# huggingface/parler-tts

Measured on NVIDIA H100. Metric: audio codec tokens/sec (all codebooks), higher is better.
Workload: dtype bf16

## Files before the change

include/ptts_b200.h:

```cpp
#ifndef PTTS_B200_H
#define PTTS_B200_H

#include <stdint.h>

#ifdef __cplusplus
extern "C" {
#endif

#define PTTS_OK 0
#define PTTS_EINVAL 1
#define PTTS_ECUDA 2
#define PTTS_ESTATE 3

#define PTTS_BF16 0
#define PTTS_F32 1
#define PTTS_I64 2
#define PTTS_I32 3

#define PTTS_HEAD_DIM 64

typedef struct ptts_decoder_config {
  int32_t hidden_size;
  int32_t num_layers;
  int32_t num_heads;
// ... 89 lines not shown
               float* out_token_nll, float* out_logits, float* out_codebook_sums, void* stream);

int ptts_decode_forward(ptts_session* s, void* stream);

int ptts_sample(ptts_session* s, const int64_t* forced_tokens, void* stream);

int ptts_decode_steps(ptts_session* s, int32_t n_steps, void* stream);

int ptts_generate_set_sampling_ext(ptts_session* s, const ptts_sampling_ext* ext);

int ptts_generate_set_outputs(ptts_session* s, float* logits, float* scores, int32_t first_step, int32_t n_steps,
                              int64_t step_stride);

int ptts_generate_set_probes(ptts_session* s, void* self_attn, void* cross_attn, void* hidden, int32_t first_step, int32_t n_steps,
                             int64_t self_ld, int64_t self_step, int64_t cross_step, int64_t hidden_step);

int ptts_session_logits(ptts_session* s, float** out);
int ptts_session_scores(ptts_session* s, float** out);
int ptts_session_raw_ids(ptts_session* s, int64_t** out, int32_t* ld);
int ptts_session_state(ptts_session* s, int32_t** out);
int ptts_session_launches(ptts_session* s, int64_t* out);
int ptts_session_fused(ptts_session* s, int32_t* out);
int ptts_session_set_profile(ptts_session* s, void* buf);

int ptts_delay_build(const int64_t* input_ids, int32_t BK, int32_t seq_len, int32_t num_codebooks,
                     int64_t bos, int64_t pad, int32_t max_length, int64_t* pattern_mask, void* stream);
int ptts_delay_apply(const int64_t* input_ids, int32_t BK, int32_t seq_len, int64_t ld_ids,
                     const int64_t* pattern_mask, int64_t ld_mask, int64_t* out, void* stream);
int ptts_logits_processor(const int64_t* input_ids, int32_t BK, int32_t seq_len, int64_t ld_ids,
                          float* scores, int32_t V, int64_t eos, int32_t num_codebooks,
                          int64_t* first_unfinished, void* stream);
int ptts_op_sample_phase(ptts_session* s, int32_t n_ctas, void* stream);
int ptts_op_linear2(const ptts_decoder_config* cfg, const void* blob, int32_t tensor_id, int32_t index,
                    const void* x, int32_t M, int32_t use_ln, int32_t epilogue ,
                    const void* residual, void* y, int32_t path, float* row_stats, void* stream);
int ptts_op_linear(const ptts_decoder_config* cfg, const void* blob, int32_t tensor_id, int32_t index,
                   const void* x, int32_t M, int32_t use_ln, int32_t epilogue, const void* residual, void* y, void* stream);
int ptts_op_attention(int32_t dtype, int32_t B, int32_t nh, int32_t nkv, int32_t q_len, int32_t past_len, int32_t cross,
                      int32_t kv_len, int32_t capacity, int32_t rope, const void* rope_cos, const void* rope_sin, const void* qkv,
                      void* kcache, void* vcache, const int32_t* key_mask, int32_t mask_len, int32_t prefill_sweep, void* out,
                      void* stream);

int ptts_op_attention_probs(int32_t dtype, int32_t B, int32_t nh, int32_t nkv, int32_t q_len, int32_t past_len, int32_t cross,
                            int32_t kv_len, int32_t capacity, int32_t rope, const void* rope_cos, const void* rope_sin, const void* q,
                            int64_t ldq, const void* kcache, const int32_t* key_mask, int32_t mask_len, void* out, void* stream);

// ... 34 lines not shown
```

parler_tts_b200/_lib.py:

```python
from __future__ import annotations
import ctypes as C
import os

import torch

_HERE = os.path.dirname(os.path.abspath(__file__))
LIB_PATH = os.environ.get("PTTS_LIB") or os.path.join(_HERE, "csrc", "libptts_b200.so")

BF16, F32, I64, I32 = 0, 1, 2, 3
OK, EINVAL, ECUDA, ESTATE = 0, 1, 2, 3


class DecoderConfigC(C.Structure):
    _fields_ = [(n, C.c_int32) for n in (
        "hidden_size", "num_layers", "num_heads", "num_kv_heads", "num_cross_kv_heads", "ffn_dim", "vocab_size",
        "num_codebooks", "max_positions", "rope", "activation", "dtype", "bos_token_id", "pad_token_id",
        "eos_token_id")] + [("rope_theta", C.c_float), ("layer_norm_eps", C.c_float)]


class GenParamsC(C.Structure):
    _fields_ = [("max_length", C.c_int32), ("min_new_tokens", C.c_int32), ("do_sample", C.c_int32),
                ("top_k", C.c_int32), ("top_p", C.c_float), ("temperature", C.c_float), ("seed", C.c_uint64),
                ("suppress_special", C.c_int32), ("codebook_size", C.c_int32),
                ("row_base", C.c_int32), ("input_len", C.c_int32)]
# ... 26 lines not shown
    "ptts_session_create": (C.c_int, [C.POINTER(DecoderConfigC), _VP, _VP, _I64, _I32, _I32, _I32, _I32, C.POINTER(_VP)]),
    "ptts_workspace_bytes2": (C.c_int, [C.POINTER(DecoderConfigC), _I32, _I32, _I32, _I32, _I32, C.POINTER(_I64)]),
    "ptts_session_create2": (C.c_int, [C.POINTER(DecoderConfigC), _VP, _VP, _I64, _I32, _I32, _I32, _I32, _I32, C.POINTER(_VP)]),
    "ptts_session_destroy": (C.c_int, [_VP]),
    "ptts_generate_begin": (C.c_int, [_VP, C.POINTER(GenParamsC), _VP]),
    "ptts_generate_begin_ids": (C.c_int, [_VP, C.POINTER(GenParamsC), _VP, _I32, _VP]),
    "ptts_generate_set_sampling_ext": (C.c_int, [_VP, C.POINTER(SamplingExtC)]),
    "ptts_generate_set_outputs": (C.c_int, [_VP, _VP, _VP, _I32, _I32, _I64]),
    "ptts_generate_set_probes": (C.c_int, [_VP, _VP, _VP, _VP, _I32, _I32, _I64, _I64, _I64, _I64]),
    "ptts_prefill": (C.c_int, [_VP, _VP, _VP, _VP, _VP, _VP]),
    "ptts_lm_heads_rowmajor_bytes": (C.c_int, [C.POINTER(DecoderConfigC), C.POINTER(_I64)]),
    "ptts_lm_heads_rowmajor_pack": (C.c_int, [C.POINTER(DecoderConfigC), _VP, _VP, _VP]),
    "ptts_score": (C.c_int, [_VP, _VP, _VP, _VP, _VP, _VP, _VP, _I32, _VP, _VP, _VP, _VP, _VP]),
    "ptts_decode_forward": (C.c_int, [_VP, _VP]),
    "ptts_sample": (C.c_int, [_VP, _VP, _VP]),
    "ptts_decode_steps": (C.c_int, [_VP, _I32, _VP]),
    "ptts_session_logits": (C.c_int, [_VP, C.POINTER(_VP)]),
    "ptts_session_scores": (C.c_int, [_VP, C.POINTER(_VP)]),
    "ptts_session_raw_ids": (C.c_int, [_VP, C.POINTER(_VP), C.POINTER(_I32)]),
    "ptts_session_state": (C.c_int, [_VP, C.POINTER(_VP)]),
    "ptts_session_launches": (C.c_int, [_VP, C.POINTER(_I64)]),
    "ptts_session_fused": (C.c_int, [_VP, C.POINTER(_I32)]),
    "ptts_session_set_profile": (C.c_int, [_VP, _VP]),
    "ptts_delay_build": (C.c_int, [_VP, _I32, _I32, _I32, _I64, _I64, _I32, _VP, _VP]),
    "ptts_delay_apply": (C.c_int, [_VP, _I32, _I32, _I64, _VP, _I64, _VP, _VP]),
    "ptts_logits_processor": (C.c_int, [_VP, _I32, _I32, _I64, _VP, _I32, _I64, _I32, _VP, _VP]),
    "ptts_op_sample_phase": (C.c_int, [_VP, _I32, _VP]),
    "ptts_op_linear": (C.c_int, [C.POINTER(DecoderConfigC), _VP, _I32, _I32, _VP, _I32, _I32, _I32, _VP, _VP, _VP]),
    "ptts_op_linear2": (C.c_int, [C.POINTER(DecoderConfigC), _VP, _I32, _I32, _VP, _I32, _I32, _I32, _VP, _VP, _I32, _VP, _VP]),
    "ptts_op_attention": (C.c_int, [_I32, _I32, _I32, _I32, _I32, _I32, _I32, _I32, _I32, _I32, _VP, _VP, _VP, _VP, _VP, _VP,
                                    _I32, _I32, _VP, _VP]),
    "ptts_op_attention_probs": (C.c_int, [_I32, _I32, _I32, _I32, _I32, _I32, _I32, _I32, _I32, _I32, _VP, _VP, _VP, _I64, _VP,
                                          _VP, _I32, _VP, _VP]),
    "ptts_dac_blob_bytes": (C.c_int, [C.POINTER(DacConfigC), C.POINTER(_I64)]),
    "ptts_dac_num_tensors": (C.c_int, [C.POINTER(DacConfigC), C.POINTER(_I32)]),
    "ptts_dac_pack": (C.c_int, [C.POINTER(DacConfigC), _VP, _I32, _VP, _I32, _I64, _VP]),
    "ptts_dac_workspace_bytes": (C.c_int, [C.POINTER(DacConfigC), _I32, _I32, C.POINTER(_I64)]),
    "ptts_dac_decode": (C.c_int, [C.POINTER(DacConfigC), _VP, _VP, _I64, _VP, _I32, _I32, _VP, _VP]),
    "ptts_dac_encoder_blob_bytes": (C.c_int, [C.POINTER(DacConfigC), C.POINTER(_I64)]),
    "ptts_dac_encoder_num_tensors": (C.c_int, [C.POINTER(DacConfigC), C.POINTER(_I32)]),
    "ptts_dac_encoder_pack": (C.c_int, [C.POINTER(DacConfigC), _VP, _I32, _VP, _I32, _I64, _VP]),
    "ptts_dac_encode_workspace_bytes": (C.c_int, [C.POINTER(DacConfigC), _I32, _I32, C.POINTER(_I64)]),
    "ptts_dac_encode": (C.c_int, [C.POINTER(DacConfigC), _VP, _VP, _VP, _I64, _VP, _I32, _I32, _I32, _VP, _VP, _VP]),
}
EXPORTED_SYMBOLS = tuple(_SIGS)

# ... 52 lines not shown
```

parler_tts_b200/csrc/api.cu:

```cuda
#include <cstdarg>
#include <cstdlib>
#include <cstring>
#include <new>

#include "common.cuh"
#include "dac.h"
#include "kernels.h"
#include "layout.h"
#include "step.h"

namespace ptts {
static thread_local std::string g_err;
void set_error(const std::string& m) { g_err = m; }
int fail(int code, const char* fmt, ...) {
  char buf[1024];
  va_list ap;
  va_start(ap, fmt);
  vsnprintf(buf, sizeof(buf), fmt, ap);
  va_end(ap);
  g_err = buf;
  return code;
}
static bool env_flag(const char* name, bool dflt) {
  const char* v = getenv(name);
// ... 11 lines not shown
};

struct ProbeWindow {
  void* self_attn; void* cross_attn; void* hidden;
  int first_step, n_steps;
  int64_t self_ld, self_step, cross_step, hidden_step;
};

struct ptts_session {
  ptts_decoder_config cfg;
  DecoderLayout L;
  WorkspaceLayout W;
  const char* blob;
  char* ws;
  int sm_count;
  bool has_prompt_mask, has_enc_mask, begun, prefilled;
  ptts_gen_params gen;
  int n0;
  cudaStream_t cap_stream;
  cudaGraphExec_t exec;
  bool graph_ready;
  int64_t launches;
  long long* prof;
  DecodePath path;
  StepParams sp;
  ptts_sampling_ext ext;
  SampleOut out;
  ProbeWindow probe;
  int64_t graph_launches;
};

static const ptts_sampling_ext kExtOff = {0, 0.f, 1.f, 0.f, 0.f};
static const ptts_sampling_ext* active_ext(const ptts_session* s) {
  const ptts_sampling_ext& x = s->ext;
  const bool warp = s->gen.do_sample && (x.min_p > 0.f || x.typical_p < 1.f || x.epsilon_cutoff > 0.f || x.eta_cutoff > 0.f);
  return (x.no_repeat_ngram_size > 0 || warp) ? &s->ext : nullptr;
}
static const SampleOut* active_out(const ptts_session* s) {
  return (s->out.logits != nullptr || s->out.scores != nullptr) ? &s->out : nullptr;
}
static const ProbeWindow* active_probe(const ptts_session* s) {
  const ProbeWindow& w = s->probe;
  return (w.self_attn != nullptr || w.cross_attn != nullptr || w.hidden != nullptr) ? &w : nullptr;
}
static DecodePath decode_path(const ptts_session* s) { return active_probe(s) != nullptr ? DECODE_MULTI_KERNEL : s->path; }

// ... 201 lines not shown
  const WorkspaceLayout& W = s->W;
  if (c.dtype != PTTS_BF16 || !env_flag("PTTS_FUSED", true)) return DECODE_MULTI_KERNEL;
  if (W.B > 32 || L.K > 16 || L.H % 64 != 0 || L.F % L.H != 0) return step_declined(s, "batch > 32 rows, > 16 codebooks or an unsupported width");
  StepParams& p = s->sp;
  memset(&p, 0, sizeof(p));
  p.B = W.B; p.H = L.H; p.F = L.F; p.V = L.V; p.K = L.K; p.L = L.L; p.nh = L.nh; p.nkv = L.nkv; p.nckv = L.nckv;
  p.S = W.S; p.P = W.P; p.Tmax = W.Tmax; p.rope = c.rope; p.act = c.activation; p.qkv_rows = L.qkv_rows; p.ckv_rows = L.ckv_rows;
  p.eps = c.layer_norm_eps; p.scale = 0.125f;
  p.blob = s->blob;
  p.lay = L;
  char* ws = s->ws;
  p.x = (bf16*)(ws + W.img_x); p.qkv = (bf16*)(ws + W.qkv); p.attn = (bf16*)(ws + W.img_attn); p.qc = (bf16*)(ws + W.qc); p.hbuf = (bf16*)(ws + W.img_h);
  p.logits = (float*)(ws + W.logits);
  p.cross_kv = ws + W.cross_kv; p.cross_layer_stride = W.cross_layer_stride;
  p.self_kv = ws + W.self_kv; p.self_layer_stride = W.self_layer_stride;
  p.prompt_mask = s->has_prompt_mask ? (const int*)(ws + W.prompt_mask) : nullptr;
  p.enc_mask = s->has_enc_mask ? (const int*)(ws + W.enc_mask) : nullptr;
  p.sa = sample_args(s);
  p.bar = ((Ctrl*)(ws + W.ctrl))->bar;
  p.progress = (int*)(ws + W.progress);
  if (const char* why = plan_decode_step(p, s->sm_count)) return step_declined(s, why);
  p.do_sample_phase = 1;
  p.prof = s->prof;
  p.cl_x = (bf16*)(ws + W.cl_x); p.cl_attn = (bf16*)(ws + W.cl_attn); p.cl_h = (bf16*)(ws + W.cl_h);
  const char* mode = getenv("PTTS_STEP");
  if (L.cl_NC > 0 && !(mode && strcmp(mode, "legacy") == 0) && cluster_step_available(p)) return DECODE_CLUSTER;
  return DECODE_STEP;
}

int ptts_generate_begin_ids(ptts_session* s, const ptts_gen_params* gen, const int64_t* input_ids, int32_t n0, void* stream) {
  PTTS_REQUIRE(s && gen, "null argument");
  PTTS_REQUIRE(n0 >= 1 && n0 <= s->W.max_input, "generate: %d decoder input columns, the session takes 1 .. %d", n0, s->W.max_input);
  PTTS_REQUIRE(input_ids != nullptr || n0 == 1, "generate: input_ids is required for %d input columns", n0);
  PTTS_REQUIRE(gen->max_length >= 2, "generate: max_length must be >= 2, got %d", gen->max_length);
  PTTS_REQUIRE(gen->max_length <= s->W.raw_ld, "generate: max_length %d exceeds the session's capacity %lld", gen->max_length, (long long)s->W.raw_ld);
  PTTS_REQUIRE(!gen->do_sample || gen->temperature > 0.f, "`temperature` has to be a strictly positive float, got %f", gen->temperature);
  PTTS_REQUIRE(gen->top_k >= 0, "`top_k` has to be a non-negative integer");
  PTTS_REQUIRE(s->cfg.eos_token_id >= 0 && s->cfg.eos_token_id < s->cfg.vocab_size, "eos_token_id out of vocabulary");
  PTTS_REQUIRE(n0 < gen->max_length, "generate: %d input columns leave nothing to generate within max_length %d", n0, gen->max_length);
  cudaStream_t st = (cudaStream_t)stream;
  s->gen = *gen;
  s->gen.input_len = n0;
  s->n0 = n0;
  s->ext = kExtOff;
  s->out = SampleOut{};
  if (active_probe(s) && s->exec) { cudaGraphExecDestroy(s->exec); s->exec = nullptr; s->graph_ready = false; }
// ... 375 lines not shown
    ce = cudaGraphInstantiate(&s->exec, graph, 0);
    cudaGraphDestroy(graph);
    if (ce != cudaSuccess) return fail(PTTS_ECUDA, "graph instantiate failed: %s", cudaGetErrorString(ce));
    s->graph_ready = true;
  }
  for (int i = 0; i < n_steps; i++) PTTS_CHECK_CUDA(cudaGraphLaunch(s->exec, st));
  s->launches += s->graph_launches * n_steps;
  return PTTS_OK;
}

int ptts_session_logits(ptts_session* s, float** out) { PTTS_REQUIRE(s && out, "null"); *out = (float*)(s->ws + s->W.logits); return PTTS_OK; }
int ptts_session_scores(ptts_session* s, float** out) { PTTS_REQUIRE(s && out, "null"); *out = (float*)(s->ws + s->W.scores); return PTTS_OK; }
int ptts_session_raw_ids(ptts_session* s, int64_t** out, int32_t* ld) {
  PTTS_REQUIRE(s && out && ld, "null");
  *out = (int64_t*)(s->ws + s->W.raw_ids);
  *ld = (int32_t)s->W.raw_ld;
  return PTTS_OK;
}
int ptts_session_state(ptts_session* s, int32_t** out) { PTTS_REQUIRE(s && out, "null"); *out = (int32_t*)(s->ws + s->W.ctrl); return PTTS_OK; }
int ptts_session_set_profile(ptts_session* s, void* buf) {
  PTTS_REQUIRE(s, "null");
  s->prof = (long long*)buf;
  s->sp.prof = s->prof;
  return PTTS_OK;
}
int ptts_session_fused(ptts_session* s, int32_t* out) { PTTS_REQUIRE(s && out, "null"); *out = s->path; return PTTS_OK; }
int ptts_session_launches(ptts_session* s, int64_t* out) { PTTS_REQUIRE(s && out, "null"); *out = s->launches; return PTTS_OK; }

int ptts_delay_build(const int64_t* input_ids, int32_t BK, int32_t seq_len, int32_t num_codebooks, int64_t bos, int64_t pad,
                     int32_t max_length, int64_t* pattern_mask, void* stream) {
  PTTS_REQUIRE(input_ids && pattern_mask, "null argument");
  PTTS_REQUIRE(num_codebooks > 0 && BK > 0 && BK % num_codebooks == 0 && seq_len > 0 && max_length > 0, "delay_build: bad shape");
  return launch_delay_build(input_ids, BK, seq_len, num_codebooks, bos, pad, max_length, pattern_mask, (cudaStream_t)stream);
}
int ptts_delay_apply(const int64_t* input_ids, int32_t BK, int32_t seq_len, int64_t ld_ids, const int64_t* pattern_mask,
                     int64_t ld_mask, int64_t* out, void* stream) {
  PTTS_REQUIRE(input_ids && pattern_mask && out, "null argument");
  PTTS_REQUIRE(BK > 0 && seq_len > 0 && ld_mask >= seq_len && ld_ids >= seq_len, "delay_apply: mask shorter than ids");
  return launch_delay_apply(input_ids, BK, seq_len, ld_ids, pattern_mask, ld_mask, out, (cudaStream_t)stream);
}
int ptts_logits_processor(const int64_t* input_ids, int32_t BK, int32_t seq_len, int64_t ld_ids, float* scores, int32_t V,
                          int64_t eos, int32_t num_codebooks, int64_t* first_unfinished, void* stream) {
  PTTS_REQUIRE(input_ids && scores && first_unfinished, "null argument");
  return launch_logits_processor(input_ids, BK, seq_len, ld_ids, scores, V, eos, num_codebooks, first_unfinished, (cudaStream_t)stream);
}

// ... 406 lines not shown
```

parler_tts_b200/csrc/sample_core.cuh:

```cuda
#pragma once
#include "common.cuh"
#include "kernels.h"

namespace ptts {

__device__ __forceinline__ uint32_t fkey(float f) {
  uint32_t u = __float_as_uint(f);
  return (u & 0x80000000u) ? ~u : (u | 0x80000000u);
}

__device__ __forceinline__ void philox_round(uint32_t (&c)[4], uint32_t k0, uint32_t k1) {
  const uint32_t hi0 = __umulhi(0xD2511F53u, c[0]), lo0 = 0xD2511F53u * c[0];
  const uint32_t hi1 = __umulhi(0xCD9E8D57u, c[2]), lo1 = 0xCD9E8D57u * c[2];
  c[0] = hi1 ^ c[1] ^ k0; c[1] = lo1; c[2] = hi0 ^ c[3] ^ k1; c[3] = lo0;
}
__device__ __forceinline__ float philox_uniform(uint64_t seed, uint32_t row, uint32_t col) {
  uint32_t c[4] = {row, col, 0x5054u, 0x5453u};
  uint32_t k0 = (uint32_t)seed, k1 = (uint32_t)(seed >> 32);
#pragma unroll
  for (int i = 0; i < 10; i++) { philox_round(c, k0, k1); k0 += 0x9E3779B9u; k1 += 0xBB67AE85u; }
  return (float)(c[0] >> 8) * (1.0f / 16777216.0f);
}


// ... 434 lines not shown
    const int still_unfinished = t_unf && !done;
    p.unfinished[my_row] = still_unfinished;
    int nxt = t;
    if (g.max_length >= 2 * p.K - 1) {
      const bool is_bos = cur_len <= k;
      const bool is_pad = (cur_len - k) >= (g.max_length - p.K + 1);
      if (is_bos || is_pad) nxt = (is_bos ? p.bos : 0) + (is_pad ? p.pad : 0);
      else if (g.input_len > 1 && cur_len - g.input_len < k) nxt = (int)p.prefix_cells[(size_t)my_row * (p.K - 1) + (cur_len - g.input_len)];
    }
    p.cur_ids[my_row] = nxt;
    if (still_unfinished) atomicAdd(&p.ctrl->n_unfinished, 1);
  }
  __syncthreads();
}

template <int ITEMS>
__device__ __forceinline__ void sample_row_cta(const SampleArgs& p, const ptts_gen_params& g, const int64_t* __restrict__ forced,
                                               int row, int cur_len) {
  sample_rows_cta<ITEMS, 1>(p, g, forced, row, 0, row + 1, cur_len);
}

template <int ITEMS>
__device__ __forceinline__ void sample_all_rows_cta(const SampleArgs& p, const ptts_gen_params& g, int cta, int n_ctas, int n_rows, int cur_len) {
  if (n_rows <= n_ctas) {
    if (cta < n_rows) sample_rows_cta<ITEMS, 1>(p, g, nullptr, cta, n_ctas, n_rows, cur_len);
  } else {
    for (int row0 = cta; row0 < n_rows; row0 += 3 * n_ctas) sample_rows_cta<ITEMS, 3>(p, g, nullptr, row0, n_ctas, n_rows, cur_len);
  }
}

}
```

parler_tts_b200/csrc/step.h:

```cpp
#pragma once
#include "common.cuh"
#include "kernels.h"
#include "layout.h"

namespace ptts {

struct StepParams {
  int B, H, F, V, K, L, nh, nkv, nckv, S, P, Tmax, rope, act, qkv_rows, ckv_rows;
  float eps, scale;
  const char* blob;
  DecoderLayout lay;
  bf16 *x, *qkv, *attn, *qc, *hbuf;
  float* logits;
  char* cross_kv; int64_t cross_layer_stride;
  char* self_kv; int64_t self_layer_stride;
  const int* prompt_mask;
  const int* enc_mask;
  SampleArgs sa;
  unsigned* bar;
  int nt_qkv, nt_h, nt_fc1, nt_heads;
  int nbuf;
  int64_t tile_region_bytes;
  int64_t wbuf_offset;
  int do_sample_phase;
  int sample_items;
  int* progress;
  int n_steps;
  long long* prof;
  bf16 *cl_x, *cl_attn, *cl_h;
};

const char* plan_decode_step(StepParams& p, int grid);
int launch_decode_step(const StepParams& p, int grid, cudaStream_t st);
bool cluster_step_available(const StepParams& p);
int launch_decode_step_cluster(const StepParams& p, cudaStream_t st);
int cluster_pack_layer(const DecoderLayout& L, char* layer, cudaStream_t st);

}
```

parler_tts_b200/csrc/step2.cu:

```cuda
#include "attn_core.cuh"
#include "common.cuh"
#include "kernels.h"
#include "ln_stats.cuh"
#include "sample_core.cuh"
#include "ptx.cuh"
#include "step.h"
#include "step_common.cuh"
#include <type_traits>

namespace ptts {
namespace cl {

constexpr int C = 2;
constexpr int V = 8;
constexpr int THREADS = 256;
constexpr int ROWS = 32;
constexpr int HROWS = 8;
constexpr int ATT_SMEM = attn_decode_smem_per_warp<bf16>();
constexpr int PROF_STRIDE = 16;
constexpr int QMAX = 6;
constexpr int OFF_STATS = 256, OFF_PART = 512, OFF_RES = 2560, OFF_CVEC = 3584;
constexpr int HDR = 5632;
constexpr int WB_BYTES = 65536;
constexpr int R_OFF = HDR + 2 * WB_BYTES;
constexpr int R_BYTES = 92160;
constexpr int QKV_OFF = R_BYTES - 2048;
constexpr int SMEM_BYTES = R_OFF + R_BYTES;
static_assert(SMEM_BYTES + 1024 <= 227 * 1024, "cluster step kernel shared memory");
static_assert(ROWS * (1024 / 2 + 8) * 2 + V * (256 + ROWS * 34 * 4) <= R_BYTES, "fc1 plan");
static_assert(HROWS * (1024 / 2 + 8) * 2 + V * C * (32 + 4 * 96 * 4) <= QKV_OFF, "QKV plan");
constexpr int ATT_STAGE = 2 * 32 * HD * 2;
constexpr int ATT_REST = ATT_SMEM - ATT_STAGE;
constexpr int ATT_S0_QKV = 34 * 1024;
constexpr int ATT_S0_QC = QKV_OFF - V * ATT_STAGE;
constexpr int ATT_S0_WB = WB_BYTES - ATT_STAGE;
static_assert(HROWS * (1024 / 2 + 8) * 2 + V * C * (32 + 4 * 96 * 4) <= ATT_S0_QKV && ATT_S0_QKV + 6 * ATT_STAGE <= QKV_OFF, "attention plan: QKV stages in R");
static_assert(HROWS * (1024 / 2 + 8) * 2 + V * C * (32 + 4 * 32 * 4) <= ATT_S0_QC, "attention plan: q_cross stages in R");
static_assert(2 * ATT_REST <= ATT_S0_QC && 2 * ATT_REST <= ATT_S0_QKV && 6 * ATT_REST <= ATT_S0_WB, "attention plan: second stages");
static_assert(6 * 8 * (1024 / 2) * 2 <= ATT_S0_WB && 16384 + 4 * 128 * 4 <= ATT_S0_WB, "attention plan: QKV weight jobs, out-proj job + pair merge");
static_assert(ROWS * (4096 / 4 + 8) * 2 + V * (256 + ROWS * 8 * 4) <= R_BYTES, "fc2 plan");

__device__ __forceinline__ void mbar_wait(uint64_t* bar, uint32_t parity, int what) {
  uint32_t ok, spins = 0;
  do {
    ok = mbar_try_wait_cluster(bar, parity);
    if (!ok && ++spins > (1u << 22)) { printf("ptts: cluster step mbarrier timeout (cta %d, barrier kind %d)\n", (int)blockIdx.x, what); __trap(); }
  } while (!ok);
}
__device__ __forceinline__ void st_async(uint32_t dst_cluster_addr, float v, uint32_t bar_cluster_addr) {
  asm volatile("st.async.shared::cluster.mbarrier::complete_tx::bytes.b32 [%0], %1, [%2];"
               ::"r"(dst_cluster_addr), "r"(__float_as_uint(v)), "r"(bar_cluster_addr) : "memory");
}
__device__ __forceinline__ void st_async(uint32_t dst_cluster_addr, float2 v, uint32_t bar_cluster_addr) {
  asm volatile("st.async.shared::cluster.mbarrier::complete_tx::bytes.v2.f32 [%0], {%1, %2}, [%3];"
               ::"r"(dst_cluster_addr), "f"(v.x), "f"(v.y), "r"(bar_cluster_addr) : "memory");
}
__device__ __forceinline__ uint32_t mapa(uint32_t addr, uint32_t rank) { uint32_t r; asm volatile("mapa.shared::cluster.u32 %0, %1, %2;" : "=r"(r) : "r"(addr), "r"(rank)); return r; }
__device__ __forceinline__ uint32_t cluster_rank() { uint32_t r; asm volatile("mov.u32 %0, %%cluster_ctarank;" : "=r"(r)); return r; }
__device__ __forceinline__ void cluster_arrive() { asm volatile("barrier.cluster.arrive.release.aligned;" ::: "memory"); }
__device__ __forceinline__ void cluster_wait() { asm volatile("barrier.cluster.wait.acquire.aligned;" ::: "memory"); }
__device__ __forceinline__ void cluster_arrive_reuse() { asm volatile("barrier.cluster.arrive.relaxed.aligned;" ::: "memory"); }

__host__ __device__ __forceinline__ int kslice(int kt) { return (kt & 7) >> 2; }
__host__ __device__ __forceinline__ int klocal(int kt) { return ((kt >> 3) << 2) | (kt & 3); }
__host__ __device__ __forceinline__ int kglobal(int rank, int lk) { return ((lk >> 2) << 3) | (rank << 2) | (lk & 3); }

template <int QN, int MT, bool STATS, bool ACC = false>
__device__ __forceinline__ void mma_slice(float (&out)[2][6][4], RowStatFrag& rst, const bf16* xs, int apitch, const uint4* wb, int KT, int kt0,
                                          int kt_end, int lrow, int lcol) {
  float acc[MT][QN][4];
#pragma unroll
  for (int a = 0; a < MT; a++)
#pragma unroll
    for (int j = 0; j < QN; j++)
#pragma unroll
      for (int e = 0; e < 4; e++) acc[a][j][e] = ACC ? out[a][j][e] : 0.f;
  for (int kt = kt0; kt < kt_end; kt += 4) {
    uint32_t a[MT][2][4];
#pragma unroll
// ... 5 lines not shown
      for (int mt = 0; mt < MT; mt++) { row_stat_mma(rst, mt, a[mt][0]); row_stat_mma(rst, mt, a[mt][1]); }
    }
#pragma unroll
    for (int j = 0; j < QN; j++) {
      const uint4 w = wb[((size_t)j * KT + kt) * 32];
#pragma unroll
      for (int mt = 0; mt < MT; mt++) {
        mma_bf16_16816(acc[mt][j], a[mt][0], w.x, w.y);
        mma_bf16_16816(acc[mt][j], a[mt][1], w.z, w.w);
      }
    }
  }
#pragma unroll
  for (int mt = 0; mt < MT; mt++)
#pragma unroll
    for (int j = 0; j < QN; j++)
#pragma unroll
      for (int e = 0; e < 4; e++) out[mt][j][e] = acc[mt][j][e];
}

enum { PH_QKV = 0, PH_O = 1, PH_QC = 2, PH_OC = 3, PH_FC1 = 4, PH_FC2 = 5 };
constexpr int JOBS_PER_LAYER = 9;
constexpr int QKV_JOBS = 4;

__device__ __forceinline__ bool weight_job(const StepParams& p, int j, int cta, int rank, const char*& src, uint32_t& bytes) {
  const int nl = JOBS_PER_LAYER * p.L;
  if (j < nl) {
    const int l = j / JOBS_PER_LAYER, jl = j - JOBS_PER_LAYER * l;
    const int ph = jl < QKV_JOBS ? 0 : jl - (QKV_JOBS - 1);
    const int64_t idx = (ph == PH_QKV || ph == PH_QC) ? (int64_t)(cta >> 3) * C + rank : (int64_t)cta;
    const int64_t sz = p.lay.cp_slice[ph];
    bytes = (uint32_t)(ph == PH_QKV ? sz / QKV_JOBS : sz);
    src = p.blob + p.lay.layer0 + p.lay.layer_stride * l + p.lay.cp[ph] + idx * sz + (ph == PH_QKV ? jl * (sz / QKV_JOBS) : 0);
    return true;
  }
  const int task = cta + (int)gridDim.x * (j - nl);
  const int ntasks = p.K * p.V / 32;
  if (task >= ntasks) return false;
  bytes = (uint32_t)(4 * p.H * 16);
  src = p.blob + p.lay.heads + (int64_t)task * bytes;
  return true;
}

template <int ITEMS>
__global__ void __launch_bounds__(THREADS, 1) decode_step_cluster_kernel(const __grid_constant__ StepParams p) {
  extern __shared__ __align__(128) unsigned char smem[];
  Ctrl* ctrl = p.sa.ctrl;
  if (p.prof != nullptr && blockIdx.x == 0 && threadIdx.x == 0) p.prof[(size_t)(6 * p.L + 2) * PROF_STRIDE + 3] = clock64();
  if (ctrl->active == 0) return;
  int cur_len = ctrl->cur_len;
  const unsigned gen = (unsigned)ctrl->launch_gen;
  int pos = p.P + cur_len - 1;
  const int tid = threadIdx.x, warp = tid >> 5, lane = tid & 31;
  const int H = p.H, F = p.F, B = p.B;
  const int rank = (int)cluster_rank(), peer = rank ^ 1;
  const int cta = (int)blockIdx.x;
  const int cluster = cta >> 1;
  const int head = cluster >> 2, rblk = cluster & 3;
  const int Ks = H / C, KsF = F / 4;
  const int pitch = Ks + 8, pitchF = KsF + 8;
  const int qe = F / p.nh / 64;
  const int dgrp = warp & 1, e4 = warp >> 1;

// ... 3 lines not shown
  uint64_t* attbars = reinterpret_cast<uint64_t*>(smem + 128);
  float* stats = reinterpret_cast<float*>(smem + OFF_STATS);
  float* part = reinterpret_cast<float*>(smem + OFF_PART);
  float* res_s = reinterpret_cast<float*>(smem + OFF_RES);
  float* cvec = reinterpret_cast<float*>(smem + OFF_CVEC);
  unsigned char* Rg = smem + R_OFF;
  const uint32_t peer_xbar = mapa(smem_u32(xbar), (uint32_t)peer);
  uint32_t par_a = 0, par_w = 0, par_x = 0, att_parity = 0;

  if (tid == 0) {
    mbar_init<1>(abar); mbar_init<1>(&wbar[0]); mbar_init<1>(&wbar[1]); mbar_init<1>(xbar);
    asm volatile("fence.mbarrier_init.release.cluster;" ::: "memory");
  }
  attention_decode_init_warp(attbars + 2 * warp, lane);
  cluster_arrive(); cluster_wait();
  unsigned* const bar_ctr = p.bar + (gen & 1u);
  unsigned bar_target = 0u;
  if (cta == 0 && tid == 0) p.bar[(gen + 1u) & 1u] = 0u;

  const char* blob = p.blob;
  long long* const prof0 = (p.prof != nullptr && cta == 0) ? p.prof : nullptr;
  long long* prof = prof0;
  prof_mark(prof, 0);

  auto issue_weight_job = [&](int j) {
    const char* src; uint32_t bytes;
    if (!weight_job(p, j, cta, rank, src, bytes)) return;
    mbar_expect_tx(&wbar[j & 1], bytes);
    bulk_g2s_evict_first(smem + HDR + (j & 1) * WB_BYTES, src, bytes, &wbar[j & 1]);
  };
  __shared__ int s_next_active;
  const int n_steps = (p.do_sample_phase && p.n_steps > 1 && prof0 == nullptr) ? p.n_steps : 1;
  int unfinished_prev = 0;
#pragma unroll 1
  for (int it = 0; it < n_steps; it++) {
  pos = p.P + cur_len - 1;
  prof = prof0;
  cluster_arrive_reuse();
  if (tid == 0) { issue_weight_job(0); issue_weight_job(1); }

  bf16* const x_img = p.cl_x;
  bf16* const a_img = p.cl_attn;
  bf16* const h_img = p.cl_h;
  const int x_slice_elems = ROWS * pitch, h_slice_elems = ROWS * pitchF;
  auto h_offset = [&](int n) {
    const int lk = klocal(n >> 5), kq = KsF >> 5;
    return (size_t)(2 * kslice(n >> 5) + lk / kq) * h_slice_elems + (lk % kq) * 32 + (n & 31);
  };
  const int xo_slice = kslice(cta >> 2), xo_col = klocal(cta >> 2) * 32 + (cta & 3) * 8;

  {
    const int row = tid >> 3, f = tid & 7, n = cta * 8 + f;
    const float v = row < B ? embed_value(p, row, n, pos) : 0.f;
    res_s[row * 8 + f] = v;
    x_img[(size_t)xo_slice * x_slice_elems + row * pitch + xo_col + f] = __float2bfloat16_rn(v);
  }
  prof_mark(prof, 6);
  auto request_slice = [&](const bf16* img_slice, uint32_t bytes) {
    fence_proxy_async_smem();
    mbar_expect_tx(abar, bytes);
    bulk_g2s(Rg, img_slice, bytes, abar);
  };
  auto slice_of = [&](int sub, const bf16*& img, uint32_t& bytes) {
    if (sub == PH_QKV || sub == PH_QC) { img = x_img + (size_t)rank * x_slice_elems + (size_t)(HROWS * rblk) * pitch; bytes = (uint32_t)(HROWS * pitch * 2); }
    else if (sub == PH_O || sub == PH_OC) { img = a_img + (size_t)rank * x_slice_elems; bytes = (uint32_t)(x_slice_elems * 2); }
    else if (sub == PH_FC1) { img = x_img + (size_t)rank * x_slice_elems; bytes = (uint32_t)(x_slice_elems * 2); }
    else { img = h_img + (size_t)(2 * rank) * h_slice_elems; bytes = (uint32_t)(h_slice_elems * 2); }
  };
  {
    const bf16* nimg; uint32_t nbytes;
    slice_of(PH_QKV, nimg, nbytes);
    bar_target = grid_sync(bar_ctr, bar_target, -1, false, nullptr, [&]() { request_slice(nimg, nbytes); });
  }
  prof_mark(prof, 7);

  const int lrow = (lane & 7) + ((lane >> 3) & 1) * 8, lcol = (lane >> 4) * 8;
  const int g = lane >> 2, t4 = lane & 3;
  const int n_phases = 6 * p.L;

  const int att_row = HROWS * rblk + 4 * rank + (warp >> 1);
  const int att_slice = kslice(2 * head), att_col = klocal(2 * head) * 32;

#pragma unroll 1
  for (int ph = 0; ph < n_phases; ph++) {
    const int l = ph / 6, sub = ph - 6 * l;
    prof = prof0 ? prof0 + (size_t)(ph + 1) * PROF_STRIDE : nullptr;
    prof_mark(prof, 0);
    const char* lb = blob + p.lay.layer0 + p.lay.layer_stride * l;
    const bool rowpart = (sub == PH_QKV || sub == PH_QC);
    const bool has_ln = (sub == PH_QKV || sub == PH_QC || sub == PH_FC1);
    const int q = (sub == PH_QKV) ? 6 : (sub == PH_QC ? 2 : (sub == PH_FC1 ? qe : 1));
    const int Nc = 4 * q * 8;
    const int KT = (sub == PH_FC2 ? KsF : Ks) >> 5;
    const int apitch = (sub == PH_FC2) ? pitchF : pitch;
    const int act_bytes = (rowpart ? HROWS : ROWS) * apitch * 2;
    const int RS = (q == 1) ? 8 : 8 * q + 2;
    const int blk = rowpart ? 32 + 4 * 16 * q * 4 : 256 + ROWS * RS * 4;
// ... 21 lines not shown
      else if (sub == PH_QC) { c1 = reinterpret_cast<const float*>(lb + p.lay.c_qc); ntot = H; }
      else { c1 = reinterpret_cast<const float*>(lb + p.lay.c_fc1); ntot = F; }
      const int nown = rowpart ? Nc : 8 * q;
      if (tid < nown) {
        int n;
        if (sub == PH_QKV) n = (tid >> 6) * (p.nh * HD) + head * HD + (tid & 63);
        else if (sub == PH_QC) n = head * HD + tid;
        else n = cta * 8 * q + tid;
        cv1 = c1[n];
        cv2 = c1[ntot + n];
      }
    }

    auto wait_job = [&](int j) {
      mbar_wait(&wbar[j & 1], (par_w >> (j & 1)) & 1u, 1);
      par_w ^= 1u << (j & 1);
    };
    auto ring = [&](int j) { return reinterpret_cast<const uint4*>(smem + HDR + (j & 1) * WB_BYTES) + lane; };
    wait_job(j0);
    if (sub == PH_QKV) wait_job(j0 + 1);
    mbar_wait(abar, par_a, 0);
    par_a ^= 1u;
    prof_mark(prof, 1);
    float acc[2][QMAX][4];
    RowStatFrag rst;
    row_stat_zero(rst);
    {
      const bf16* xs = reinterpret_cast<const bf16*>(Rg);
      if (rowpart) {
        auto head_pass = [&](auto pass_tag) {
          constexpr int P = decltype(pass_tag)::value;
          const int u = 2 * P + dgrp;
          float t[2][QMAX][4];
          if (sub == PH_QKV) mma_slice<6, 1, P == 0>(t, rst, xs, apitch, ring(j0 + u), KT, e4, KT, lrow & 7, lcol);
          else mma_slice<2, 1, P == 0>(t, rst, xs, apitch, ring(j0) + (size_t)(2 * u) * KT * 32, KT, e4, KT, lrow & 7, lcol);
          const int d = g >> 2;
          const uint32_t slot = (uint32_t)((8 * rank + warp) * blk);
          if (P == 0) {
            cluster_wait();
            if (dgrp == 0) {
              const uint32_t so = slot + 8 * (g & 3);
              if (t4 == 0) put(d, so, rst.s1[0][0]);
              if (t4 == (g >> 1)) put(d, so + 4, (g & 1) ? rst.sq[0][0][1] : rst.sq[0][0][0]);
            }
          }
#pragma unroll
// ... 165 lines not shown
    }
    prof_mark(prof, 6);
    if (p.prof != nullptr && l == p.L / 2 && tid == 0) {
      unsigned long long ns;
      asm volatile("mov.u64 %0, %%globaltimer;" : "=l"(ns));
      p.prof[(size_t)(n_phases + 4) * PROF_STRIDE + sub * (int)gridDim.x + cta] = (long long)ns;
    }

    const bool last = (ph + 1 == n_phases);
    const bf16* nimg; uint32_t nbytes;
    if (last) { nimg = x_img; nbytes = (uint32_t)(C * x_slice_elems * 2); }
    else slice_of((sub + 1) % 6, nimg, nbytes);
    const int held_job = sub == PH_QKV ? j0 + QKV_JOBS + 1 : (sub == PH_QC || sub == PH_OC) ? j0 + 2 : -1;
    bar_target = grid_sync(bar_ctr, bar_target, ph, false, nullptr, [&]() {
      request_slice(nimg, nbytes);
      if (held_job >= 0) issue_weight_job(held_job);
    });
    prof_mark(prof, 7);
  }
  cluster_wait();

  prof = prof0 ? prof0 + (size_t)(n_phases + 1) * PROF_STRIDE : nullptr;
  prof_mark(prof, 0);
  {
    const int ntasks = p.K * p.V / 32;
    const float* c1 = reinterpret_cast<const float*>(blob + p.lay.c_heads);
    const float* c2 = c1 + p.K * p.V;
    mbar_wait(abar, par_a, 3);
    par_a ^= 1u;
    const bf16* xs = reinterpret_cast<const bf16*>(Rg);
    const int KTH = H >> 5;
    auto ktile = [&](int kt) { return xs + (size_t)kslice(kt) * x_slice_elems + klocal(kt) * 32; };
    {
      RowStatFrag rst;
      row_stat_zero(rst);
      for (int kt = warp; kt < KTH; kt += 8) {
        const bf16* sl = ktile(kt);
#pragma unroll
        for (int mt = 0; mt < 2; mt++)
#pragma unroll
          for (int j = 0; j < 2; j++) {
            uint32_t a[4];
            ldmatrix_x4(a, sl + (size_t)(mt * 16 + lrow) * pitch + j * 16 + lcol);
            row_stat_mma(rst, mt, a);
          }
      }
      row_stat_store(rst, part, warp, lane);
      __syncthreads();
      row_stat_finalize(part, H, ROWS, p.eps, stats);
      __syncthreads();
    }
    prof_mark(prof, 1);
    constexpr int HRS = 40;
    int job = JOBS_PER_LAYER * p.L;
    for (int task = cta; task < ntasks; task += (int)gridDim.x, job++) {
      mbar_wait(&wbar[job & 1], (par_w >> (job & 1)) & 1u, 4);
      par_w ^= 1u << (job & 1);
      float acc[2][4][4];
#pragma unroll
      for (int a = 0; a < 2; a++)
#pragma unroll
        for (int j = 0; j < 4; j++)
#pragma unroll
          for (int e = 0; e < 4; e++) acc[a][j][e] = 0.f;
      unsigned char* wbuf = smem + HDR + (job & 1) * WB_BYTES;
      const uint4* wb = reinterpret_cast<const uint4*>(wbuf) + lane;
      for (int kt = warp; kt < KTH; kt += 8) {
        const bf16* sl = ktile(kt);
        uint32_t a[2][2][4];
#pragma unroll
        for (int mt = 0; mt < 2; mt++)
#pragma unroll
          for (int j = 0; j < 2; j++) ldmatrix_x4(a[mt][j], sl + (size_t)(mt * 16 + lrow) * pitch + j * 16 + lcol);
#pragma unroll
        for (int j = 0; j < 4; j++) {
          const uint4 w = wb[((size_t)j * KTH + kt) * 32];
#pragma unroll
          for (int mt = 0; mt < 2; mt++) {
            mma_bf16_16816(acc[mt][j], a[mt][0], w.x, w.y);
            mma_bf16_16816(acc[mt][j], a[mt][1], w.z, w.w);
          }
        }
      }
      __syncthreads();
      float* red = reinterpret_cast<float*>(wbuf);
#pragma unroll
      for (int mt = 0; mt < 2; mt++)
#pragma unroll
        for (int j = 0; j < 4; j++) {
          float* base = red + ((size_t)warp * 32 + mt * 16 + g) * HRS + j * 8 + 2 * t4;
          *reinterpret_cast<float2*>(base) = make_float2(acc[mt][j][0], acc[mt][j][1]);
          *reinterpret_cast<float2*>(base + 8 * HRS) = make_float2(acc[mt][j][2], acc[mt][j][3]);
        }
      __syncthreads();
      {
        const int er = tid >> 3, ec = tid & 7;
        if (er < B) {
          const float mean = stats[2 * er], rstd = stats[2 * er + 1];
#pragma unroll
          for (int j = 0; j < 4; j++) {
            const int cidx = j * 8 + ec, n = task * 32 + cidx;
            float v = 0.f;
#pragma unroll
            for (int w = 0; w < 8; w++) v += red[((size_t)w * 32 + er) * HRS + cidx];
            p.logits[(size_t)er * p.K * p.V + n] = DT<bf16>::rnd(rstd * (v - mean * c1[n]) + c2[n]);
          }
        }
      }
      __syncthreads();
      if (tid == 32) {
        fence_proxy_async_smem();
        issue_weight_job(job + 2);
      }
    }
  }
  prof_mark(prof, 6);
  bar_target = grid_sync(bar_ctr, bar_target, n_phases, true);
  prof = prof0 ? prof0 + (size_t)(n_phases + 2) * PROF_STRIDE : nullptr;
  prof_mark(prof, 0);
  if (p.do_sample_phase) {
    const ptts_gen_params gp = *p.sa.gen;
    const int BK = B * p.K;
    sample_phase<ITEMS>(p.sa, gp, BK, cur_len);
    prof_mark(prof, 1);
    bar_target = grid_sync(bar_ctr, bar_target, n_phases + 1, true, nullptr, [&]() {
      const int tot = *reinterpret_cast<volatile int*>(&ctrl->n_unfinished);
      s_next_active = (tot - unfinished_prev > 0) ? 1 : 0;
      unfinished_prev = tot;
    });
    prof_mark(prof, 2);
  }
  bool go_on = false;
  if (p.do_sample_phase) {
    const int act = s_next_active;
    if (cta == 0 && tid == 0) {
      ctrl->cur_len = cur_len + 1;
      ctrl->active = act;
      ctrl->steps_run += 1;
    }
    go_on = act != 0;
    cur_len += 1;
  }
  if (!go_on) break;
  }
  if (cta == 0 && tid == 0) {
    if (p.do_sample_phase) ctrl->n_unfinished = 0;
    ctrl->launch_gen = (int)(gen + 1u);
  }
}

__global__ void cluster_pack_kernel(const uint4* __restrict__ src, uint4* __restrict__ dst, int ph, int nh, int ntc, int kts, int KT_src) {
  const int64_t tile = blockIdx.x;
  const int ktl = (int)(tile % kts);
  const int j = (int)((tile / kts) % ntc);
  const int slice = (int)(tile / ((int64_t)kts * ntc));
  const int rank = slice & 1, owner = slice >> 1;
  int n_tile;
  if (ph == PH_QKV) n_tile = (j >> 3) * (nh * 8) + owner * 8 + (j & 7);
  else n_tile = owner * ntc + j;
  const int kt = kglobal(rank, ktl);
  dst[tile * 32 + threadIdx.x] = src[((int64_t)n_tile * KT_src + kt) * 32 + threadIdx.x];
}

}

int cluster_pack_layer(const DecoderLayout& L, char* layer, cudaStream_t st) {
// ... 63 lines not shown
```

parler_tts_b200/csrc/step_common.cuh:

```cuda
#pragma once
#include "attn_core.cuh"
#include "common.cuh"
#include "sample_core.cuh"
#include "step.h"

namespace ptts {

__device__ __forceinline__ float embed_value(const StepParams& p, int row, int col, int pos) {
  const bf16* tables = reinterpret_cast<const bf16*>(p.blob + p.lay.embed);
  float v = 0.f;
#pragma unroll 1
  for (int k0 = 0; k0 < p.K; k0 += 8) {
    float ev[8];
#pragma unroll
    for (int k = 0; k < 8; k++)
      if (k0 + k < p.K) ev[k] = __bfloat162float(tables[((size_t)(k0 + k) * (p.V + 1) + p.sa.cur_ids[row * p.K + k0 + k]) * p.H + col]);
#pragma unroll
    for (int k = 0; k < 8; k++)
      if (k0 + k < p.K) v = (k0 + k == 0) ? ev[k] : DT<bf16>::rnd(v + ev[k]);
  }
  if (!p.rope) v = DT<bf16>::rnd(v + __bfloat162float(reinterpret_cast<const bf16*>(p.blob + p.lay.pos)[(size_t)pos * p.H + col]));
  return v;
}

__device__ __forceinline__ AttnArgs decode_attn_args(const StepParams& p, int l, int pos, bool cross) {
  AttnArgs a{};
  a.ctrl = nullptr; a.B = p.B; a.nh = p.nh; a.q_len = 1;
  a.past_from_ctrl = 0; a.past_len = pos; a.prefix = p.P;
  a.rope = p.rope; a.rope_cos = p.blob + p.lay.rope_cos; a.rope_sin = p.blob + p.lay.rope_sin; a.scale = p.scale;
  if (!cross) {
    char* kc = p.self_kv + p.self_layer_stride * l;
    a.kcache = kc; a.vcache = kc + (size_t)p.B * p.nkv * p.Tmax * HD * 2;
    a.kv_b_stride = (int64_t)p.nkv * p.Tmax * HD; a.kv_h_stride = (int64_t)p.Tmax * HD; a.kv_t_stride = HD;
    a.key_mask = p.prompt_mask; a.mask_len = p.P; a.mask_ld = p.P;
    a.nkv = p.nkv; a.cross = 0; a.kv_len = 0; a.kv_capacity = p.Tmax;
  } else {
    char* ck = p.cross_kv + p.cross_layer_stride * l;
    a.kcache = ck; a.vcache = ck + (size_t)p.B * p.nckv * p.S * HD * 2;
    a.kv_b_stride = (int64_t)p.nckv * p.S * HD; a.kv_h_stride = (int64_t)p.S * HD; a.kv_t_stride = HD;
    a.key_mask = p.enc_mask; a.mask_len = p.S; a.mask_ld = p.S;
    a.nkv = p.nckv; a.cross = 1; a.kv_len = p.S; a.kv_capacity = p.S;
// ... 11 lines not shown
```

Measured before the change: 252,000.

## Prefetch next-step weights during heads, balance head chunks, simplify sampling loop

The first two weight jobs of the next decode step are now issued right after the LM-heads phase, so they overlap with sampling and the grid sync instead of being issued at step start. LM-head tiles are split into contiguous, evenly sized chunks per CTA, with a guard for partial chunks. The multi-row sampling path is replaced by a plain strided per-row loop, and embedding gathers are batched 16 at a time. It also adds optional per-token globaltimer profiling, plus an mbarrier drain on early exit to keep the prefetch consistent.

Result: no change. 253,000, median of 6 (+0.4%).

```diff
diff --git a/include/ptts_b200.h b/include/ptts_b200.h
--- a/include/ptts_b200.h
+++ b/include/ptts_b200.h
@@ -135,6 +135,7 @@
 int ptts_session_launches(ptts_session* s, int64_t* out);
 int ptts_session_fused(ptts_session* s, int32_t* out);
 int ptts_session_set_profile(ptts_session* s, void* buf);
+int ptts_session_set_token_profile(ptts_session* s, void* buf);
 
 int ptts_delay_build(const int64_t* input_ids, int32_t BK, int32_t seq_len, int32_t num_codebooks,
                      int64_t bos, int64_t pad, int32_t max_length, int64_t* pattern_mask, void* stream);
diff --git a/parler_tts_b200/_lib.py b/parler_tts_b200/_lib.py
--- a/parler_tts_b200/_lib.py
+++ b/parler_tts_b200/_lib.py
@@ -72,6 +72,7 @@
     "ptts_session_launches": (C.c_int, [_VP, C.POINTER(_I64)]),
     "ptts_session_fused": (C.c_int, [_VP, C.POINTER(_I32)]),
     "ptts_session_set_profile": (C.c_int, [_VP, _VP]),
+    "ptts_session_set_token_profile": (C.c_int, [_VP, _VP]),
     "ptts_delay_build": (C.c_int, [_VP, _I32, _I32, _I32, _I64, _I64, _I32, _VP, _VP]),
     "ptts_delay_apply": (C.c_int, [_VP, _I32, _I32, _I64, _VP, _I64, _VP, _VP]),
     "ptts_logits_processor": (C.c_int, [_VP, _I32, _I32, _I64, _VP, _I32, _I64, _I32, _VP, _VP]),
diff --git a/parler_tts_b200/csrc/api.cu b/parler_tts_b200/csrc/api.cu
--- a/parler_tts_b200/csrc/api.cu
+++ b/parler_tts_b200/csrc/api.cu
@@ -57,6 +57,7 @@
   bool graph_ready;
   int64_t launches;
   long long* prof;
+  long long* tok_prof;
   DecodePath path;
   StepParams sp;
   ptts_sampling_ext ext;
@@ -304,6 +305,7 @@
   if (const char* why = plan_decode_step(p, s->sm_count)) return step_declined(s, why);
   p.do_sample_phase = 1;
   p.prof = s->prof;
+  p.tok_prof = s->tok_prof;
   p.cl_x = (bf16*)(ws + W.cl_x); p.cl_attn = (bf16*)(ws + W.cl_attn); p.cl_h = (bf16*)(ws + W.cl_h);
   const char* mode = getenv("PTTS_STEP");
   if (L.cl_NC > 0 && !(mode && strcmp(mode, "legacy") == 0) && cluster_step_available(p)) return DECODE_CLUSTER;
@@ -725,6 +727,12 @@
   PTTS_REQUIRE(s, "null");
   s->prof = (long long*)buf;
   s->sp.prof = s->prof;
+  return PTTS_OK;
+}
+int ptts_session_set_token_profile(ptts_session* s, void* buf) {
+  PTTS_REQUIRE(s, "null");
+  s->tok_prof = (long long*)buf;
+  s->sp.tok_prof = s->tok_prof;
   return PTTS_OK;
 }
 int ptts_session_fused(ptts_session* s, int32_t* out) { PTTS_REQUIRE(s && out, "null"); *out = s->path; return PTTS_OK; }
diff --git a/parler_tts_b200/csrc/sample_core.cuh b/parler_tts_b200/csrc/sample_core.cuh
--- a/parler_tts_b200/csrc/sample_core.cuh
+++ b/parler_tts_b200/csrc/sample_core.cuh
@@ -480,11 +480,7 @@
 
 template <int ITEMS>
 __device__ __forceinline__ void sample_all_rows_cta(const SampleArgs& p, const ptts_gen_params& g, int cta, int n_ctas, int n_rows, int cur_len) {
-  if (n_rows <= n_ctas) {
-    if (cta < n_rows) sample_rows_cta<ITEMS, 1>(p, g, nullptr, cta, n_ctas, n_rows, cur_len);
-  } else {
-    for (int row0 = cta; row0 < n_rows; row0 += 3 * n_ctas) sample_rows_cta<ITEMS, 3>(p, g, nullptr, row0, n_ctas, n_rows, cur_len);
-  }
-}
-
-}
+  for (int row = cta; row < n_rows; row += n_ctas) sample_rows_cta<ITEMS, 1>(p, g, nullptr, row, 0, n_rows, cur_len);
+}
+
+}
diff --git a/parler_tts_b200/csrc/step.h b/parler_tts_b200/csrc/step.h
--- a/parler_tts_b200/csrc/step.h
+++ b/parler_tts_b200/csrc/step.h
@@ -27,6 +27,7 @@
   int* progress;
   int n_steps;
   long long* prof;
+  long long* tok_prof;
   bf16 *cl_x, *cl_attn, *cl_h;
 };
 
diff --git a/parler_tts_b200/csrc/step2.cu b/parler_tts_b200/csrc/step2.cu
--- a/parler_tts_b200/csrc/step2.cu
+++ b/parler_tts_b200/csrc/step2.cu
@@ -18,6 +18,20 @@
 constexpr int HROWS = 8;
 constexpr int ATT_SMEM = attn_decode_smem_per_warp<bf16>();
 constexpr int PROF_STRIDE = 16;
+constexpr int TOK_STRIDE = 16;
+enum {
+  TS_START = 0,
+  TS_EMBED = 1,
+  TS_OPEN = 2,
+  TS_QKV = 3,
+  TS_HEADS = 4,
+  TS_HEADS_DONE = 5,
+  TS_HEADS_LAST = 6,
+  TS_SAMPLE = 7,
+  TS_SAMPLE_DONE = 8,
+  TS_SAMPLE_LAST = 9,
+  TS_NEXT = 10,
+};
 constexpr int QMAX = 6;
 constexpr int OFF_STATS = 256, OFF_PART = 512, OFF_RES = 2560, OFF_CVEC = 3584;
 constexpr int HDR = 5632;
@@ -55,6 +69,7 @@
   asm volatile("st.async.shared::cluster.mbarrier::complete_tx::bytes.v2.f32 [%0], {%1, %2}, [%3];"
                ::"r"(dst_cluster_addr), "f"(v.x), "f"(v.y), "r"(bar_cluster_addr) : "memory");
 }
+__device__ __forceinline__ unsigned long long globaltimer() { unsigned long long ns; asm volatile("mov.u64 %0, %%globaltimer;" : "=l"(ns)); return ns; }
 __device__ __forceinline__ uint32_t mapa(uint32_t addr, uint32_t rank) { uint32_t r; asm volatile("mapa.shared::cluster.u32 %0, %1, %2;" : "=r"(r) : "r"(addr), "r"(rank)); return r; }
 __device__ __forceinline__ uint32_t cluster_rank() { uint32_t r; asm volatile("mov.u32 %0, %%cluster_ctarank;" : "=r"(r)); return r; }
 __device__ __forceinline__ void cluster_arrive() { asm volatile("barrier.cluster.arrive.release.aligned;" ::: "memory"); }
@@ -106,6 +121,13 @@
 enum { PH_QKV = 0, PH_O = 1, PH_QC = 2, PH_OC = 3, PH_FC1 = 4, PH_FC2 = 5 };
 constexpr int JOBS_PER_LAYER = 9;
 constexpr int QKV_JOBS = 4;
+
+__device__ __forceinline__ int head_chunk(const StepParams& p, int cta, int i, int& t0) {
+  const int nt_all = p.K * p.V / 8, G = (int)gridDim.x;
+  const int hi = (int)((int64_t)(cta + 1) * nt_all / G);
+  t0 = (int)((int64_t)cta * nt_all / G) + 4 * i;
+  return min(4, hi - t0);
+}
 
 __device__ __forceinline__ bool weight_job(const StepParams& p, int j, int cta, int rank, const char*& src, uint32_t& bytes) {
   const int nl = JOBS_PER_LAYER * p.L;
@@ -118,11 +140,11 @@
     src = p.blob + p.lay.layer0 + p.lay.layer_stride * l + p.lay.cp[ph] + idx * sz + (ph == PH_QKV ? jl * (sz / QKV_JOBS) : 0);
     return true;
   }
-  const int task = cta + (int)gridDim.x * (j - nl);
-  const int ntasks = p.K * p.V / 32;
-  if (task >= ntasks) return false;
-  bytes = (uint32_t)(4 * p.H * 16);
-  src = p.blob + p.lay.heads + (int64_t)task * bytes;
+  int t0;
+  const int nt = head_chunk(p, cta, j - nl, t0);
+  if (nt <= 0) return false;
+  bytes = (uint32_t)(nt * p.H * 16);
+  src = p.blob + p.lay.heads + (int64_t)t0 * p.H * 16;
   return true;
 }
 
@@ -172,6 +194,12 @@
   long long* const prof0 = (p.prof != nullptr && cta == 0) ? p.prof : nullptr;
   long long* prof = prof0;
   prof_mark(prof, 0);
+  auto tok_mark = [&](int slot) {
+    if (p.tok_prof == nullptr || tid != 0) return;
+    long long* row = p.tok_prof + (size_t)cur_len * TOK_STRIDE;
+    if (slot == TS_HEADS_LAST || slot == TS_SAMPLE_LAST) atomicMax(reinterpret_cast<unsigned long long*>(row + slot), globaltimer());
+    else if (cta == 0) row[slot] = (long long)globaltimer();
+  };
 
   auto issue_weight_job = [&](int j) {
     const char* src; uint32_t bytes;
@@ -186,8 +214,9 @@
   for (int it = 0; it < n_steps; it++) {
   pos = p.P + cur_len - 1;
   prof = prof0;
+  tok_mark(TS_START);
   cluster_arrive_reuse();
-  if (tid == 0) { issue_weight_job(0); issue_weight_job(1); }
+  if (tid == 0 && it == 0) { issue_weight_job(0); issue_weight_job(1); }
 
   bf16* const x_img = p.cl_x;
   bf16* const a_img = p.cl_attn;
@@ -206,6 +235,7 @@
     x_img[(size_t)xo_slice * x_slice_elems + row * pitch + xo_col + f] = __float2bfloat16_rn(v);
   }
   prof_mark(prof, 6);
+  tok_mark(TS_EMBED);
   auto request_slice = [&](const bf16* img_slice, uint32_t bytes) {
     fence_proxy_async_smem();
     mbar_expect_tx(abar, bytes);
@@ -223,6 +253,7 @@
     bar_target = grid_sync(bar_ctr, bar_target, -1, false, nullptr, [&]() { request_slice(nimg, nbytes); });
   }
   prof_mark(prof, 7);
+  tok_mark(TS_OPEN);
 
   const int lrow = (lane & 7) + ((lane >> 3) & 1) * 8, lcol = (lane >> 4) * 8;
   const int g = lane >> 2, t4 = lane & 3;
@@ -290,6 +321,7 @@
     mbar_wait(abar, par_a, 0);
     par_a ^= 1u;
     prof_mark(prof, 1);
+    if (ph == 0) tok_mark(TS_QKV);
     float acc[2][QMAX][4];
     RowStatFrag rst;
     row_stat_zero(rst);
@@ -501,8 +533,8 @@
 
   prof = prof0 ? prof0 + (size_t)(n_phases + 1) * PROF_STRIDE : nullptr;
   prof_mark(prof, 0);
+  tok_mark(TS_HEADS);
   {
-    const int ntasks = p.K * p.V / 32;
     const float* c1 = reinterpret_cast<const float*>(blob + p.lay.c_heads);
     const float* c2 = c1 + p.K * p.V;
     mbar_wait(abar, par_a, 3);
@@ -532,7 +564,10 @@
     prof_mark(prof, 1);
     constexpr int HRS = 40;
     int job = JOBS_PER_LAYER * p.L;
-    for (int task = cta; task < ntasks; task += (int)gridDim.x, job++) {
+    for (int i = 0;; i++, job++) {
+      int t0;
+      const int nt = head_chunk(p, cta, i, t0);
+      if (nt <= 0) break;
       mbar_wait(&wbar[job & 1], (par_w >> (job & 1)) & 1u, 4);
       par_w ^= 1u << (job & 1);
       float acc[2][4][4];
@@ -553,11 +588,13 @@
           for (int j = 0; j < 2; j++) ldmatrix_x4(a[mt][j], sl + (size_t)(mt * 16 + lrow) * pitch + j * 16 + lcol);
 #pragma unroll
         for (int j = 0; j < 4; j++) {
-          const uint4 w = wb[((size_t)j * KTH + kt) * 32];
-#pragma unroll
-          for (int mt = 0; mt < 2; mt++) {
-            mma_bf16_16816(acc[mt][j], a[mt][0], w.x, w.y);
-            mma_bf16_16816(acc[mt][j], a[mt][1], w.z, w.w);
+          if (j < nt) {
+            const uint4 w = wb[((size_t)j * KTH + kt) * 32];
+#pragma unroll
+            for (int mt = 0; mt < 2; mt++) {
+              mma_bf16_16816(acc[mt][j], a[mt][0], w.x, w.y);
+              mma_bf16_16816(acc[mt][j], a[mt][1], w.z, w.w);
+            }
           }
         }
       }
@@ -578,7 +615,8 @@
           const float mean = stats[2 * er], rstd = stats[2 * er + 1];
 #pragma unroll
           for (int j = 0; j < 4; j++) {
-            const int cidx = j * 8 + ec, n = task * 32 + cidx;
+            if (j >= nt) break;
+            const int cidx = j * 8 + ec, n = t0 * 8 + cidx;
             float v = 0.f;
 #pragma unroll
             for (int w = 0; w < 8; w++) v += red[((size_t)w * 32 + er) * HRS + cidx];
@@ -593,21 +631,28 @@
       }
     }
   }
+  if (tid == 32 && it + 1 < n_steps) { fence_proxy_async_smem(); issue_weight_job(0); issue_weight_job(1); }
   prof_mark(prof, 6);
+  tok_mark(TS_HEADS_DONE);
+  tok_mark(TS_HEADS_LAST);
   bar_target = grid_sync(bar_ctr, bar_target, n_phases, true);
   prof = prof0 ? prof0 + (size_t)(n_phases + 2) * PROF_STRIDE : nullptr;
   prof_mark(prof, 0);
+  tok_mark(TS_SAMPLE);
   if (p.do_sample_phase) {
     const ptts_gen_params gp = *p.sa.gen;
     const int BK = B * p.K;
     sample_phase<ITEMS>(p.sa, gp, BK, cur_len);
     prof_mark(prof, 1);
+    tok_mark(TS_SAMPLE_DONE);
+    tok_mark(TS_SAMPLE_LAST);
     bar_target = grid_sync(bar_ctr, bar_target, n_phases + 1, true, nullptr, [&]() {
       const int tot = *reinterpret_cast<volatile int*>(&ctrl->n_unfinished);
       s_next_active = (tot - unfinished_prev > 0) ? 1 : 0;
       unfinished_prev = tot;
     });
     prof_mark(prof, 2);
+    tok_mark(TS_NEXT);
   }
   bool go_on = false;
   if (p.do_sample_phase) {
@@ -620,7 +665,10 @@
     go_on = act != 0;
     cur_len += 1;
   }
-  if (!go_on) break;
+  if (!go_on) {
+    if (tid == 0 && it + 1 < n_steps) { mbar_wait(&wbar[0], par_w & 1u, 1); mbar_wait(&wbar[1], (par_w >> 1) & 1u, 1); }
+    break;
+  }
   }
   if (cta == 0 && tid == 0) {
     if (p.do_sample_phase) ctrl->n_unfinished = 0;
diff --git a/parler_tts_b200/csrc/step_common.cuh b/parler_tts_b200/csrc/step_common.cuh
--- a/parler_tts_b200/csrc/step_common.cuh
+++ b/parler_tts_b200/csrc/step_common.cuh
@@ -10,13 +10,13 @@
   const bf16* tables = reinterpret_cast<const bf16*>(p.blob + p.lay.embed);
   float v = 0.f;
 #pragma unroll 1
-  for (int k0 = 0; k0 < p.K; k0 += 8) {
-    float ev[8];
+  for (int k0 = 0; k0 < p.K; k0 += 16) {
+    float ev[16];
 #pragma unroll
-    for (int k = 0; k < 8; k++)
+    for (int k = 0; k < 16; k++)
       if (k0 + k < p.K) ev[k] = __bfloat162float(tables[((size_t)(k0 + k) * (p.V + 1) + p.sa.cur_ids[row * p.K + k0 + k]) * p.H + col]);
 #pragma unroll
-    for (int k = 0; k < 8; k++)
+    for (int k = 0; k < 16; k++)
       if (k0 + k < p.K) v = (k0 + k == 0) ? ev[k] : DT<bf16>::rnd(v + ev[k]);
   }
   if (!p.rope) v = DT<bf16>::rnd(v + __bfloat162float(reinterpret_cast<const bf16*>(p.blob + p.lay.pos)[(size_t)pos * p.H + col]));
```
